# BinFuPKU/CollaborativeFilteringUsingTensorflow

Hardware: AMD Instinct MI355X
Metric: BPR triplets/sec/GPU (d=64) + achieved HBM GB/s; NDCG@10 vs ref (higher is better)
Workload: dtype f32

## Files before the change

collaborativefilteringusingtensorflow_amd/csrc/cf_device.h:

```cpp
#pragma once
#include <hip/hip_runtime.h>
#include <stdint.h>
#include "cf_kernels.h"

namespace cfk {

__host__ __device__ __forceinline__ uint64_t mix64(uint64_t z) {
    z += 0x9E3779B97F4A7C15ull;
    z = (z ^ (z >> 30)) * 0xBF58476D1CE4E5B9ull;
    z = (z ^ (z >> 27)) * 0x94D049BB133111EBull;
    return z ^ (z >> 31);
}

__device__ __forceinline__ uint64_t uniform_below(uint64_t h, uint64_t n) {
    return __umul64hi(h, n);
}

__host__ __device__ __forceinline__ uint64_t perm_rounds(uint64_t x, const PermKey& p) {
#pragma unroll
    for (int r = 0; r < 3; ++r) {
        x = (x ^ p.k[r]) & p.mask;
        x = (x * p.m[r]) & p.mask;
        x ^= x >> p.shift;
    }
    return x;
}

__host__ __device__ __forceinline__ uint64_t permute(uint64_t x, const PermKey& p) {
    do {
        x = perm_rounds(x, p);
    } while (x >= p.n);
    return x;
}

struct PermInv {
    uint64_t mi[3];
};
__host__ __device__ __forceinline__ uint64_t perm_mul_inverse(uint64_t m) {
// ... 87 lines not shown
```

collaborativefilteringusingtensorflow_amd/csrc/cf_engine.cpp:

```cpp
#include <hip/hip_runtime.h>

#include <algorithm>
#include <atomic>
#include <cmath>
#include <cstdio>
#include <cstring>
#include <string>
#include <utility>
#include <vector>

#include "../../include/cf_engine.h"
#include "cf_device.h"
#include "cf_host.h"
#include "cf_kernels.h"
#include <thread>

using namespace cfk;
using namespace cfi;

namespace {
thread_local std::string g_err;
}

std::atomic<int64_t> cfi::g_live_bytes[2];
// ... 27 lines not shown
    int64_t nnz = 0;
    DevBuf<int64_t> indptr;
    DevBuf<int32_t> indices;
    DevBuf<int4> pairs;
    int spec_neg = 0;
    DevBuf<long long> slotP64;
    DevBuf<unsigned long long> GU64;
    DevBuf<int32_t> hotU;
    DevBuf<int> hot_n;
    DevBuf<unsigned long long> GV64;
    int fx_cap = 0;
    DevBuf<unsigned long long> pos_set;
    uint64_t pos_mask = 0;
    int neg_check = 0;
    int64_t nnz_set = 0;
    DevBuf<int64_t> indptr_t;
    DevBuf<int32_t> indices_t;
    std::vector<int64_t> h_indptr;
    int sorted_batches = 2;
    bool sorted_auto_off = false;
    int64_t sorted_reserve_mb = 1024;
    int epoch_sort = 0;
    int user_runs = 0;
    struct EpochOrder {
        DevBuf<int32_t> keys;
        DevBuf<int32_t> vals;
        DevBuf<char> tmp;
        int64_t epoch = -1;
        int B = 0;
        const int32_t* order = nullptr;
        DevBuf<int4> recs;
        const int4* recs_sorted = nullptr;
        bool with_recs = false;
        hipEvent_t ready = nullptr;
        bool async = false;
    } eo[2];
    hipStream_t eo_stream = nullptr;
    hipEvent_t eo_mark = nullptr;

    DevBuf<float> tab[6];
    float *U = nullptr, *V = nullptr, *b = nullptr;
    float *AU = nullptr, *AV = nullptr, *Ab = nullptr;
    DevBuf<float> GU, GV_own, Gb_own;
    float *GV = nullptr, *Gb = nullptr;
    DevBuf<float> GadvU, GadvV;
    float* GadvV_bound = nullptr;
    DevBuf<float> slotU;
    DevBuf<float> slotV;
    DevBuf<float> slotVb;
    int capU = 2, capV = 32;
    bool capU_auto = true;
    int item_recs = 0;
    DevBuf<int4> recV;
    DevBuf<int4> recVc;
    DevBuf<float> stashU, stashB;
    DevBuf<float> GVrep;
// ... 452 lines not shown
            a.fx_bad = e->fx_bad + std::min(e->fx_step++, kFxSlots - 1);
        }
    }
    a.shard_u0 = e->shard_u0;
    a.shard_u1 = e->shard_u1;
    a.plr_kind = c.plr_kind;
    a.alpha = c.alpha;
    a.beta = c.beta;
    a.gamma = c.gamma;
    a.train_bias = (c.model == CF_GBPR || (c.model == CF_PLR && c.plr_kind == CF_PLR_CPLR)) ? 1 : 0;
    a.coefs = e->coefs;
    a.xrows = e->x_rows;
    a.xgrads = e->x_grads;
    return a;
}

constexpr int64_t kSortedAutoBatches = 16;
bool sorted_batches_on(const cf_engine* e, int B) {
    if (e->sorted_batches == 0 || e->nnz > INT32_MAX || B < 1) return false;
    if (e->sorted_batches == 2 && e->sorted_auto_off) return false;
    return e->sorted_batches == 1 || e->sorted_batches == 3 || e->nnz / B >= kSortedAutoBatches;
}

struct EpochNeed {
    bool counting;
    int64_t keys, vals, recs;
    size_t tmp;
    double bytes() const { return 4.0 * (double)(keys + vals) + 16.0 * (double)recs + (double)tmp; }
};
EpochNeed epoch_need(const cf_engine* e, int B) {
    const int64_t nnz = e->nnz;
    const bool wr = e->sorted_batches != 3;
    EpochNeed n{};
    n.counting = e->epoch_sort == 0 && epoch_count_ok(nnz, B);
    if (n.counting) {
        n.recs = wr ? nnz : 0;
        n.vals = wr ? 0 : nnz;
        n.tmp = epoch_count_scratch(nnz, B);
    } else {
        n.keys = 2 * nnz;
        n.recs = wr ? 2 * nnz : 0;
        n.vals = wr ? 0 : 2 * nnz;
        n.tmp = wr ? epoch_records_scratch(nnz, (int32_t)(nnz / B)) : epoch_order_scratch(nnz, (int32_t)(nnz / B));
    }
    return n;
}
// ... 27 lines not shown
        (void)hipGetLastError();
        return true;
    }
    return (double)free_b >= more + (double)e->sorted_reserve_mb * (double)(1 << 20);
}

template <typename T>
int refit(DevBuf<T>& b, size_t need, const char* what) {
    if (b.cap >= need) return CF_OK;
    CF_HIP(hipDeviceSynchronize());
    return b.reset(need, what);
}

int compute_epoch_order(cf_engine* e, int k, int64_t epoch, int B, hipStream_t st) {
    cf_engine::EpochOrder& o = e->eo[k];
    const int64_t nnz = e->nnz;
    const bool wr = e->sorted_batches != 3;
    const EpochNeed n = epoch_need(e, B);
    CF_TRY(refit(o.keys, (size_t)n.keys, "epoch order keys"));
    CF_TRY(refit(o.vals, (size_t)n.vals, "epoch order values"));
    CF_TRY(refit(o.recs, (size_t)n.recs, "epoch order records"));
    CF_TRY(refit(o.tmp, n.tmp, "epoch order scratch"));
    const PermKey pk = make_perm_key((uint64_t)nnz, e->cfg.seed, (uint64_t)epoch);
    {
        ProfScope ps(e, CF_K_EPOCH_ORDER, st);
        if (n.counting) {
            CF_HIP(launch_epoch_count(pk, nnz, B, wr ? e->pairs.p : nullptr, wr ? o.recs.p : nullptr,
                                      wr ? nullptr : o.vals.p, o.tmp, o.tmp.cap, st));
            o.recs_sorted = wr ? o.recs.p : nullptr;
            o.order = wr ? nullptr : o.vals.p;
        } else if (wr) {
            CF_HIP(launch_epoch_records(pk, nnz, B, e->pairs, o.keys, o.recs, o.tmp, o.tmp.cap, &o.recs_sorted, st));
            o.order = nullptr;
        } else {
            CF_HIP(launch_epoch_order(pk, nnz, B, o.keys, o.vals, o.tmp, o.tmp.cap, &o.order, st));
            o.recs_sorted = nullptr;
        }
        o.with_recs = wr;
    }
    o.epoch = epoch;
    o.B = B;
    o.async = st != e->stream;
    if (o.async) CF_HIP(hipEventRecord(o.ready, st));
    return CF_OK;
}

int epoch_order(cf_engine* e, int B, const int32_t** out, const int4** recs_out) {
    if (!e->eo_stream) {
        int lo = 0, hi = 0;
        CF_HIP(hipDeviceGetStreamPriorityRange(&lo, &hi));
        CF_HIP(hipStreamCreateWithPriority(&e->eo_stream, hipStreamNonBlocking, lo));
        CF_HIP(hipEventCreateWithFlags(&e->eo_mark, hipEventDisableTiming));
        for (auto& o : e->eo) CF_HIP(hipEventCreateWithFlags(&o.ready, hipEventDisableTiming));
    }
    const int64_t ep = e->epoch;
    const bool wr = e->sorted_batches != 3;
    auto have = [&](const cf_engine::EpochOrder& o, int64_t epc) { return o.epoch == epc && o.B == B && o.with_recs == wr; };
    int k = have(e->eo[0], ep) ? 0 : have(e->eo[1], ep) ? 1 : -1;
    if (k < 0) {
        k = have(e->eo[0], ep + 1) ? 1 : 0;
        if (e->eo[k].async) CF_HIP(hipStreamWaitEvent(e->stream, e->eo[k].ready, 0));
        CF_HIP(hipEventRecord(e->eo_mark, e->side));
        CF_HIP(hipStreamWaitEvent(e->stream, e->eo_mark, 0));
        CF_TRY(compute_epoch_order(e, k, ep, B, e->stream));
        CF_HIP(hipEventRecord(e->eo_mark, e->stream));
        CF_HIP(hipStreamWaitEvent(e->side, e->eo_mark, 0));
    } else if (e->eo[k].async) {
        CF_HIP(hipStreamWaitEvent(e->stream, e->eo[k].ready, 0));
        CF_HIP(hipStreamWaitEvent(e->side, e->eo[k].ready, 0));
        e->eo[k].async = false;
    }
    *out = e->eo[k].order;
    *recs_out = e->eo[k].with_recs ? e->eo[k].recs_sorted : nullptr;
    cf_engine::EpochOrder& nx = e->eo[k ^ 1];
    if (!have(nx, ep + 1) && e->nnz / B >= 2) {
        CF_HIP(hipEventRecord(e->eo_mark, e->stream));
        CF_HIP(hipStreamWaitEvent(e->eo_stream, e->eo_mark, 0));
        CF_HIP(hipEventRecord(e->eo_mark, e->side));
        CF_HIP(hipStreamWaitEvent(e->eo_stream, e->eo_mark, 0));
        CF_TRY(compute_epoch_order(e, k ^ 1, ep + 1, B, e->eo_stream));
    }
    return CF_OK;
}

int sampler_args(cf_engine* e, int B, StepArgs* a) {
    if (!e->pairs) return fail(CF_ESTATE, "no interactions: call cf_set_interactions first");
    if ((int64_t)B > e->nnz) return fail(CF_EINVAL, "batch size exceeds the number of interactions");
    if (e->full_row_user >= 0)
        return fail(CF_EINVAL, "user " + std::to_string(e->full_row_user) +
                                   " has every item as a positive; the device sampler cannot draw a negative");
    if (e->sampler_B != B) {
        if (e->sampler_B != 0 && e->batch != 0) {
            e->epoch += 1;
            e->batch = 0;
        }
        e->sampler_B = B;
    }
    const int64_t per_epoch = e->nnz / B;
    if (e->batch >= per_epoch) {
        e->epoch += 1;
        e->batch = 0;
    }
    a->sample = 1;
    a->slot_base = (uint64_t)(e->batch * (int64_t)B);
    a->perm = make_perm_key((uint64_t)e->nnz, e->cfg.seed, (uint64_t)e->epoch);
    a->rng_key = mix64_host(e->cfg.seed ^ mix64_host((uint64_t)e->epoch * 0x9E3779B97F4A7C15ull +
                                                     0x2545F4914F6CDD1Dull));
    if (sorted_batches_on(e, B) && e->sorted_batches == 2 && !sorted_auto_fits(e, B)) e->sorted_auto_off = true;
    if (sorted_batches_on(e, B)) {
        const int32_t* ord = nullptr;
        const int4* recs = nullptr;
        const int rc = epoch_order(e, B, &ord, &recs);
        if (rc == CF_ENOMEM && e->sorted_batches == 2) {
            free_epoch_orders(e);
            e->sorted_auto_off = true;
        } else if (rc != CF_OK) {
            return rc;
        } else {
            a->order = ord;
            a->order_recs = recs;
            a->user_runs = e->user_runs && group_count(e->cfg) == 0 ? 1 : 0;
        }
    }
    e->batch += 1;
    return CF_OK;
}

static bool is_device_ptr(const void* p) {
    if (!p) return false;
    hipPointerAttribute_t attr;
    if (hipPointerGetAttributes(&attr, p) != hipSuccess) {
        (void)hipGetLastError();
        return false;
    }
    return attr.type == hipMemoryTypeDevice;
}

static int stage_device_batch(cf_engine* e, const int32_t* pairs, const int32_t* negs,
                       const int32_t* groups, int B, int k, hipStream_t st) {
    const cf_config& c = e->cfg;
    const int W = c.n_neg, G = group_count(c);
    if (!is_device_ptr(negs) || (G > 0 && !is_device_ptr(groups)))
        return fail(CF_EINVAL, "a batch must be all host or all device memory");
// ... 1912 lines not shown
        if (value < 0 || value > 2) return fail(CF_EINVAL, "topk_path must be 0, 1 or 2");
        e->topk_path = (int)value;
        return CF_OK;
    }
    if (n == "item_pieces") {
        if (value < 1 || value > 64) return fail(CF_EINVAL, "item_pieces must be 1 .. 64");
        if (e->lg_stage != 0) return fail(CF_ESTATE, "a split step is in progress");
        e->item_pieces = (int)value;
        return CF_OK;
    }
    if (n == "sorted_batches") {
        if (value < 0 || value > 3) return fail(CF_EINVAL, "sorted_batches must be 0, 1, 2 or 3");
        CF_TRY(discard_pending(e));
        e->sorted_batches = (int)value;
        e->sorted_auto_off = false;
        return CF_OK;
    }
    if (n == "user_runs") {
        if (value < 0 || value > 1) return fail(CF_EINVAL, "user_runs must be 0 or 1");
        CF_TRY(discard_pending(e));
        e->user_runs = (int)value;
        return CF_OK;
    }
    if (n == "epoch_sort") {
        if (value < 0 || value > 1) return fail(CF_EINVAL, "epoch_sort must be 0 or 1");
        CF_TRY(discard_pending(e));
        if (e->eo_stream) CF_HIP(hipStreamSynchronize(e->eo_stream));
        e->epoch_sort = (int)value;
        for (auto& o : e->eo) o.epoch = -1;
        return CF_OK;
    }
    if (n == "sorted_auto_reserve_mb") {
        if (value < 0) return fail(CF_EINVAL, "sorted_auto_reserve_mb must be >= 0");
        CF_TRY(discard_pending(e));
        e->sorted_reserve_mb = value;
        e->sorted_auto_off = false;
        return CF_OK;
    }
    if (n == "spec_neg") {
        if (value < 0 || value > 1) return fail(CF_EINVAL, "spec_neg must be 0 or 1");
        CF_TRY(discard_pending(e));
        e->spec_neg = (int)value;
        return CF_OK;
    }
    if (n == "pair_prefetch") {
        if (value != 0) return fail(CF_EINVAL, "pair_prefetch must be 0 (the prefetch was removed)");
// ... 123 lines not shown
}

int cf_step_path(cf_engine* e, int32_t B, int32_t* flags_out) {
    if (!e || !flags_out) return fail(CF_EINVAL, "null argument");
    if (B < 1) return fail(CF_EINVAL, "B must be >= 1");
    const cf_config& c = e->cfg;
    StepArgs a{};
    a.model = c.model;
    a.d = c.n_factors;
    a.W = c.n_neg;
    a.G = group_count(c);
    a.grad_path = e->grad_path;
    a.apr = (c.model == CF_AMF && e->phase == 1 && c.amf_mode == CF_AMF_APR) ? 1 : 0;
    a.B = B;
    const int kind = grad_plan(a, nullptr).kind;
    int f = 0;
    if (kind == kGradPhased || kind == kGradLds) f |= CF_PATH_PHASED;
    if (psort_active(e, B)) f |= CF_PATH_POS_SORT;
    else if (kind == kGradLds) f |= CF_PATH_LDS;
    if (e->item_recs && (!c.dense_item_apply || e->item_reduce)) f |= CF_PATH_ITEM_RECORDS;
    if (e->det) f |= CF_PATH_DETERMINISTIC;
    if (c.dense_item_apply) f |= CF_PATH_DENSE_ITEMS;
    if (e->pairs && sorted_batches_on(e, B)) f |= CF_PATH_SORTED_BATCHES;
    f |= (e->pipeline & 3) << 8;
    *flags_out = f;
    return CF_OK;
}

int cf_profile_enable(cf_engine* e, int32_t on) {
    if (!e) return fail(CF_EINVAL, "null engine");
    e->prof = on != 0;
    return CF_OK;
}

int cf_profile_read(cf_engine* e, int32_t kid, double* total_ms, int64_t* launches) {
    CF_TRY(check_engine(e));
    if (kid < 0 || kid >= CF_K_COUNT) return fail(CF_EINVAL, "bad kernel id");
    CF_HIP(hipStreamSynchronize(e->stream));
    double t = 0.0;
    for (auto& pr : e->ev[kid]) {
        float ms = 0.f;
        CF_HIP(hipEventSynchronize(pr.second));
        CF_HIP(hipEventElapsedTime(&ms, pr.first, pr.second));
        t += ms;
    }
    if (total_ms) *total_ms = t;
// ... 26 lines not shown
```

collaborativefilteringusingtensorflow_amd/csrc/cf_epoch.hip:

```cpp
#include "cf_kernels.h"
#include "cf_device.h"

namespace cfk {

namespace {

constexpr int kEpochTile = 2048;
constexpr int kEpochItems = kEpochTile / kBlock;
constexpr int kEpochWaveSpan = kEpochTile / kWavesPerBlock;
constexpr int kEpochChunkTiles = 32;

struct EpochCtx {
    uint32_t n, mask, shift, B;
    uint32_t k[3], mi[3];
    uint64_t magic;
    uint32_t nb, n_used;
    int32_t n_bins, nbits;
    int32_t xs_steps;
    int32_t pad;
    int64_t n_tiles;
};

__device__ __forceinline__ uint32_t rounds_inv32(uint32_t q, const EpochCtx& c) {
#pragma unroll
// ... 78 lines not shown
    const int64_t t0 = (int64_t)blockIdx.x * kEpochChunkTiles;
    const int64_t t1 = min(t0 + (int64_t)kEpochChunkTiles, c.n_tiles);
    for (int b = threadIdx.x; b < c.n_bins; b += kBlock) {
        int32_t run = csum[(int64_t)blockIdx.x * c.n_bins + b];
        for (int64_t g = t0; g < t1; ++g) {
            const int32_t t = cnt[g * c.n_bins + b];
            cnt[g * c.n_bins + b] = run;
            run += t;
        }
    }
}

__device__ __forceinline__ int32_t block_excl_scan(int32_t v, int32_t* wtot) {
    const int w = threadIdx.x >> 6, lane = threadIdx.x & 63;
    const int32_t inc = wave_incl_scan(v);
    if (lane == kWave - 1) wtot[w] = inc;
    __syncthreads();
    int32_t before = 0;
#pragma unroll
    for (int i = 0; i < kWavesPerBlock; ++i) before += i < w ? wtot[i] : 0;
    return before + inc - v;
}

template <bool RECS>
__global__ void __launch_bounds__(kBlock) epoch_scatter_kernel(EpochCtx c, const uint16_t* __restrict__ bins,
                                                               const int32_t* __restrict__ off,
                                                               const int4* __restrict__ pairs,
                                                               int4* __restrict__ out_recs,
                                                               int32_t* __restrict__ out_idx) {
    extern __shared__ int32_t lds[];
    const int nbn = c.n_bins;
    int32_t* stage = lds;
    int32_t* gstage = stage + kEpochTile;
    int32_t* wtot = gstage + kEpochTile;
    int32_t* wcnt = wtot + kWavesPerBlock;
    int32_t* delta = wcnt + kWavesPerBlock * nbn;
    const int tid = threadIdx.x, w = tid >> 6, lane = tid & 63;
    const uint32_t tile0 = (uint32_t)blockIdx.x * kEpochTile;
    const uint32_t qend = min(tile0 + (uint32_t)kEpochTile, c.n);
    const int tile_len = (int)(qend - tile0);
    for (int b = tid; b < kWavesPerBlock * nbn; b += kBlock) wcnt[b] = 0;
    __syncthreads();
    const uint32_t w0 = tile0 + (uint32_t)(w * kEpochWaveSpan);
    constexpr int KC = kEpochWaveSpan / kWave;
    int key[KC];
#pragma unroll
    for (int k = 0; k < KC; ++k) {
        const uint32_t q = w0 + (uint32_t)(k * kWave + lane);
        key[k] = q < qend ? (int)bins[q] : nbn;
    }
#pragma unroll
    for (int k = 0; k < KC; ++k)
// ... 38 lines not shown
        for (int bit = 0; bit < c.nbits; ++bit) {
            const bool s = (key[k] >> bit) & 1;
            const uint64_t m = __ballot(s);
            peers &= s ? m : ~m;
        }
        const int rank = __popcll(peers & below);
        if (key[k] < nbn) {
            const int32_t lp = pos[key[k]] + rank;
            if (rank == 0) pos[key[k]] = lp + __popcll(peers);
            gstage[lp] = lp + delta[key[k]];
            stage[lp] = (int32_t)(w0 + (uint32_t)(k * kWave + lane));
        }
    }
    __syncthreads();
    if (RECS) {
        int4 r[kEpochItems];
        int32_t g[kEpochItems];
#pragma unroll
        for (int i = 0; i < kEpochItems; ++i) {
            const int L = tid + i * kBlock;
            const int Lc = L < tile_len ? L : 0;
            g[i] = gstage[Lc];
            r[i] = pairs[stage[Lc]];
        }
        __builtin_amdgcn_sched_barrier(0);
#pragma unroll
        for (int i = 0; i < kEpochItems; ++i) out_recs[g[i]] = r[i];
    } else {
#pragma unroll
        for (int i = 0; i < kEpochItems; ++i) {
            const int L = tid + i * kBlock;
            if (L < tile_len) out_idx[gstage[L]] = stage[L];
        }
    }
}

EpochCtx epoch_ctx(const PermKey& p, int64_t nnz, int B) {
    EpochCtx c{};
    c.n = (uint32_t)p.n;
    c.mask = (uint32_t)p.mask;
    c.shift = p.shift;
    c.B = (uint32_t)B;
    for (int r = 0; r < 3; ++r) {
        c.k[r] = (uint32_t)p.k[r];
        c.mi[r] = (uint32_t)perm_mul_inverse(p.m[r]);
    }
// ... 12 lines not shown
    c.n_tiles = (nnz + kEpochTile - 1) / kEpochTile;
    return c;
}

int64_t n_chunks_of(int64_t n_tiles) { return (n_tiles + kEpochChunkTiles - 1) / kEpochChunkTiles; }

size_t align16(size_t x) { return (x + 15) & ~(size_t)15; }

}

bool epoch_count_ok(int64_t nnz, int B) {
    return nnz > 0 && nnz <= INT32_MAX && B > 0 && nnz / B + 1 <= kEpochMaxBins;
}

size_t epoch_count_scratch(int64_t nnz, int B) {
    if (!epoch_count_ok(nnz, B)) return 0;
    const int64_t n_bins = nnz / B + 1;
    const int64_t n_tiles = (nnz + kEpochTile - 1) / kEpochTile;
    return align16((size_t)nnz * sizeof(uint16_t)) +
           (size_t)((n_tiles + n_chunks_of(n_tiles)) * n_bins) * sizeof(int32_t);
}

hipError_t launch_epoch_count(const PermKey& p, int64_t nnz, int B, const int4* pairs, int4* out_recs,
                              int32_t* out_idx, void* tmp, size_t tmp_bytes, hipStream_t s) {
    if (!epoch_count_ok(nnz, B) || (uint64_t)nnz != p.n || p.mask > 0xFFFFFFFFull) return hipErrorInvalidValue;
    if ((pairs == nullptr) != (out_recs == nullptr) || (out_recs == nullptr) == (out_idx == nullptr))
        return hipErrorInvalidValue;
    if (tmp_bytes < epoch_count_scratch(nnz, B)) return hipErrorInvalidValue;
    const EpochCtx c = epoch_ctx(p, nnz, B);
    const int64_t n_chunks = n_chunks_of(c.n_tiles);
    uint16_t* bins = static_cast<uint16_t*>(tmp);
    int32_t* cnt = reinterpret_cast<int32_t*>(static_cast<char*>(tmp) + align16((size_t)nnz * sizeof(uint16_t)));
    int32_t* csum = cnt + c.n_tiles * c.n_bins;
    const dim3 grid((unsigned)c.n_tiles);
    const size_t lds1 = (size_t)c.n_bins * sizeof(int32_t) + kEpochTile * sizeof(uint16_t);
    hipLaunchKernelGGL(epoch_bins_kernel, grid, dim3(kBlock), lds1, s, c, bins, cnt);
    hipLaunchKernelGGL(epoch_chunk_sum_kernel, dim3((unsigned)n_chunks), dim3(kBlock), 0, s, c, cnt, csum);
    hipLaunchKernelGGL(epoch_chunk_scan_kernel, dim3((unsigned)((c.n_bins + kWavesPerBlock - 1) / kWavesPerBlock)),
                       dim3(kBlock), 0, s, c, csum, n_chunks);
    hipLaunchKernelGGL(epoch_tile_offsets_kernel, dim3((unsigned)n_chunks), dim3(kBlock), 0, s, c, cnt, csum);
    size_t lds3 = (size_t)(kWavesPerBlock + 1) * c.n_bins * sizeof(int32_t) +
                  (size_t)(2 * kEpochTile + kWavesPerBlock) * sizeof(int32_t);
    if (out_recs)
        hipLaunchKernelGGL(epoch_scatter_kernel<true>, grid, dim3(kBlock), lds3, s, c, bins, cnt, pairs, out_recs,
                           nullptr);
    else
        hipLaunchKernelGGL(epoch_scatter_kernel<false>, grid, dim3(kBlock), lds3, s, c, bins, cnt, nullptr, nullptr,
                           out_idx);
    return hipGetLastError();
}

}
```

collaborativefilteringusingtensorflow_amd/csrc/cf_kernels.h:

```cpp
#pragma once
#include <hip/hip_runtime.h>
#include <stdint.h>

namespace cfk {

constexpr int kWave = 64;
constexpr int kBlock = 256;
constexpr int kWavesPerBlock = kBlock / kWave;
constexpr int kGL = 16;
constexpr int kGroupsPerBlock = kBlock / kGL;
#ifndef CF_PAIRS_PER_GROUP
#define CF_PAIRS_PER_GROUP 2
#endif
constexpr int kPairsPerGroup = CF_PAIRS_PER_GROUP;
constexpr int kPairsPerBlock = kGroupsPerBlock * kPairsPerGroup;
constexpr int kMaxNeg = 64;
constexpr int kMaxGroup = 16;
constexpr int kMaxFactors = 256;

enum Model { BPR = 0, GBPR = 1, CML = 2, AMF = 3, PLR = 4 };

struct PermKey {
    uint64_t n;
    uint64_t mask;
// ... 20 lines not shown
    int apr_embed_done;
    int use_rank_weight;
    float n_items_f;
    int64_t n_items;
    float lr, clip_norm;
    int clip;
    int sample;
    int count_users;
    int count_items;
    int items_grad_only;
    uint64_t slot_base;
    uint64_t rng_key;
    PermKey perm;
    const int4* __restrict__ pairs;
    const int64_t* __restrict__ indptr;
    const int32_t* __restrict__ indices;
    const int64_t* __restrict__ indptr_t;
    const int32_t* __restrict__ indices_t;
    const unsigned long long* __restrict__ pos_set;
    uint64_t pos_mask;
    const int32_t* __restrict__ order;
    const int4* __restrict__ order_recs;
    int user_runs;
    int det_fx;
    long long* __restrict__ slotP64;
    unsigned long long* __restrict__ GU64;
    const int32_t* __restrict__ hotU;
    unsigned long long* __restrict__ GV64;
    int* __restrict__ fx_bad;
    int2* __restrict__ spec_ph;
    int* __restrict__ spec_n;
    float* __restrict__ U; float* __restrict__ AU; float* __restrict__ GU;
    float* __restrict__ V; float* __restrict__ AV; float* __restrict__ GV;
    float* __restrict__ b; float* __restrict__ Ab; float* __restrict__ Gb;
    int32_t* __restrict__ occU;
    int32_t* __restrict__ occV;
    int32_t* __restrict__ cntU;
    int32_t* __restrict__ cntV;
    int32_t* __restrict__ rankU;
    int32_t* __restrict__ rankV;
    float* __restrict__ slotU;
    float* __restrict__ slotV;
    int capU, capV;
    float* __restrict__ GVrep;
    int repV;
    const int32_t* __restrict__ offU;
// ... 248 lines not shown
    const int32_t* occV; const int32_t* rankV;
    const int32_t* cntU;
    int32_t* hotU;
    int* hot_n;
    const int32_t* cntV; const int32_t* cntP;
    int2* offPN;
    int32_t* srec;
    int B, W, capU;
    int64_t n_items;
    const int2* spec_ph;
    const int* spec_n;
    float* slotN;
    int32_t* cntVw;
    int d;
};
hipError_t launch_psort(const PsortArgs& a, void* tmp, size_t tmp_bytes, hipStream_t s);
size_t epoch_order_scratch(int64_t nnz, int32_t n_batches);
hipError_t launch_epoch_order(const PermKey& p, int64_t nnz, int B, int32_t* keys, int32_t* vals, void* tmp,
                              size_t tmp_bytes, const int32_t** order_out, hipStream_t s);
size_t epoch_records_scratch(int64_t nnz, int32_t n_batches);
hipError_t launch_epoch_records(const PermKey& p, int64_t nnz, int B, const int4* pairs, int32_t* keys, int4* recs,
                                void* tmp, size_t tmp_bytes, const int4** recs_out, hipStream_t s);
constexpr int kEpochMaxBins = 1024;
bool epoch_count_ok(int64_t nnz, int B);
size_t epoch_count_scratch(int64_t nnz, int B);
hipError_t launch_epoch_count(const PermKey& p, int64_t nnz, int B, const int4* pairs, int4* out_recs,
                              int32_t* out_idx, void* tmp, size_t tmp_bytes, hipStream_t s);
hipError_t launch_uncount_spec(const int2* ph, int* n, int32_t* cnt, hipStream_t s);
hipError_t launch_build_pos_set(const int4* pairs, int64_t nnz, unsigned long long* set,
                                uint64_t mask, hipStream_t s);
hipError_t launch_build_pairs(const int64_t* indptr, const int32_t* indices, int64_t n_users,
                              int4* pairs, hipStream_t s);
hipError_t launch_score(const ScoreArgs& a, hipStream_t s);
hipError_t launch_topk(const TopkArgs& a, int n_users, hipStream_t s);
hipError_t launch_fused_topk(const FusedTopkArgs& a, hipStream_t s);
hipError_t launch_xchg_pack(const XchgArgs& a, hipStream_t s);
hipError_t launch_xchg_serve(const int32_t* ids, int64_t n, int64_t u0, int32_t* cntU, int32_t* own,
                             const float* U, float* rows, int d, hipStream_t s);
hipError_t launch_xchg_accumulate(const int32_t* ids, int64_t n, int64_t u0, const float* grads,
                                  float* GU, int d, hipStream_t s);

PermKey make_perm_key(uint64_t n, uint64_t seed, uint64_t epoch);
uint64_t mix64_host(uint64_t z);

}
```

collaborativefilteringusingtensorflow_amd/csrc/cf_kernels.hip:

```cpp
#include "cf_kernels_impl.h"

namespace cfk {

__global__ void init_normal_kernel(float* __restrict__ X, int64_t n, float mean, float stddev,
                                   int truncated, uint64_t seed) {
    const int64_t t0 = (int64_t)blockIdx.x * blockDim.x + threadIdx.x;
    const int64_t nt = (int64_t)gridDim.x * blockDim.x;
    for (int64_t k = t0; k < n; k += nt) {
        uint64_t ctr = 0;
        float z;
        do {
            const uint64_t h = mix64(seed ^ mix64((uint64_t)k * 0x9E3779B97F4A7C15ull + ctr++));
            const float u1 = ((uint32_t)(h >> 40) + 0.5f) * (1.f / 16777216.f);
            const float u2 = ((uint32_t)(h & 0xFFFFFF)) * (1.f / 16777216.f);
            z = sqrtf(-2.f * logf(u1)) * cospif(2.f * u2);
        } while (truncated && fabsf(z) > 2.f);
        X[k] = mean + stddev * z;
    }
}

__global__ void fill_kernel(float* __restrict__ X, int64_t n, float v) {
    const int64_t t0 = (int64_t)blockIdx.x * blockDim.x + threadIdx.x;
    const int64_t nt = (int64_t)gridDim.x * blockDim.x;
    for (int64_t k = t0; k < n; k += nt) X[k] = v;
// ... 438 lines not shown
        const int32_t g = a.g[(int64_t)p * a.gs + k];
        int32_t v;
        if (a.sharded) {
            const bool gok = g >= 0 && g < a.total_users;
            ok = ok && gok;
            v = !gok ? 0 : (g >= a.shard_u0 && g < a.shard_u1) ? (int32_t)(g - a.shard_u0) : -1 - g;
        } else {
            const bool gok = g >= 0 && g < a.n_users;
            ok = ok && gok;
            v = gok ? g : 0;
        }
        a.occU[a.B + (int64_t)p * a.G + k] = v;
    }
    if (!ok) atomicMin(a.bad, p);
}

hipError_t launch_pack_batch(const PackArgs& a, hipStream_t s) {
    if (a.B <= 0) return hipSuccess;
    hipLaunchKernelGGL(pack_batch_kernel, dim3((a.B + kBlock - 1) / kBlock), dim3(kBlock), 0, s, a);
    return hipGetLastError();
}

uint64_t mix64_host(uint64_t z) { return mix64(z); }

PermKey make_perm_key(uint64_t n, uint64_t seed, uint64_t epoch) {
    PermKey p{};
    p.n = n;
    uint32_t bits = 1;
    while (bits < 63 && (1ull << bits) < n) ++bits;
    p.mask = (1ull << bits) - 1ull;
    p.shift = bits / 2 > 0 ? bits / 2 : 1;
    uint64_t h = mix64(seed ^ mix64(epoch + 0x5851F42D4C957F2Dull));
    for (int r = 0; r < 3; ++r) {
        h = mix64(h + (uint64_t)r);
        p.k[r] = h & p.mask;
        p.m[r] = (mix64(h ^ 0xA0761D6478BD642Full) | 1ull);
    }
    return p;
}

hipError_t launch_det_hot(const HotArgs& h, hipStream_t s) {
    const int64_t ntiles = h.n / kDetTile;
    if (ntiles <= 0) return hipSuccess;
    const dim3 grid((unsigned)(ntiles < 16384 ? ntiles : 16384)), block(kBlock);
    return with_epl(h.d, [&](auto e) {
        hipLaunchKernelGGL(det_hot_kernel<decltype(e)::value>, grid, block, 0, s, h);
// ... 5 lines not shown
```

collaborativefilteringusingtensorflow_amd/csrc/cf_kernels_impl.h:

```cpp
#pragma once
#include <algorithm>
#include <type_traits>

#include "cf_kernels.h"
#include "cf_device.h"

#ifndef CF_PREP_GL
#define CF_PREP_GL 8
#endif
#ifndef CF_PREP_CHUNKS
#define CF_PREP_CHUNKS 8
#endif
#ifndef CF_PREP_GL_W1
#define CF_PREP_GL_W1 4
#endif
#ifndef CF_PREP_CHUNKS_W1
#define CF_PREP_CHUNKS_W1 (64 / CF_PREP_GL_W1)
#endif
#ifndef CF_SORT_MIN_WAVES
#define CF_SORT_MIN_WAVES 1
#endif
#ifndef CF_SORT_TILES
#define CF_SORT_TILES 1
#endif
#ifndef CF_LDS_WAVES
#define CF_LDS_WAVES 1
#endif
#ifndef CF_LDS_WAVES_GBPR
#define CF_LDS_WAVES_GBPR 1
#endif
#ifndef CF_APPLY_NF
#define CF_APPLY_NF 4
#endif
#ifndef CF_APPLY_NF_PS
#define CF_APPLY_NF_PS 8
#endif
#ifndef CF_APPLY_MIN_WAVES
#define CF_APPLY_MIN_WAVES 1
#endif
#ifndef CF_APPLY_DETECT_WAVES
// ... 262 lines not shown
        unsafeAtomicAdd(a.Gb + r, g);
    }
}

__device__ __forceinline__ void bias_finish_pre(const StepArgs& a, int64_t r, int count, float g,
                                                int64_t slot, float b0, float ab0) {
    if (count == 1 && !a.items_grad_only) {
        const float acc = fmaf(g, g, ab0);
        a.Ab[r] = acc;
        a.b[r] = b0 - adagrad_delta(a.lr, g, acc);
    } else {
        bias_finish(a, r, count, g, slot);
    }
}

__device__ __forceinline__ float neg_log_sigmoid(float x) {
    return -logf(rcp_1p(expf(-x)));
}

__device__ __forceinline__ float softplus(float x) {
    return x > 0.f ? x + log1pf(expf(-x)) : log1pf(expf(x));
}

__device__ __forceinline__ int32_t draw_item(uint64_t key, uint64_t ctr, int64_t n_items) {
    return (int32_t)uniform_below(mix64(key + ctr), (uint64_t)n_items);
}

constexpr int kPrepGL = CF_PREP_GL;
constexpr int kPrepPairsPerBlock = kBlock / kPrepGL;
constexpr int kPrepChunks = CF_PREP_CHUNKS;
__host__ __device__ constexpr int prep_chunks(int pgl) { return pgl == kPrepGL ? kPrepChunks : CF_PREP_CHUNKS_W1; }

template <int PGL = kPrepGL>
__device__ __forceinline__ uint32_t gor8(uint32_t v) {
    if constexpr (PGL == 4 || PGL == 8) {
        v |= dpp_u<0xB1>(v);
        v |= dpp_u<0x4E>(v);
        if constexpr (PGL == 8) v |= dpp_u<0x141>(v);
        return v;
    }
#pragma unroll
    for (int o = PGL / 2; o >= 1; o >>= 1) v |= (uint32_t)__shfl_xor((int)v, o, 64);
    return v;
}
template <int PGL>
__device__ __forceinline__ int32_t gbcast(int32_t v, int k) {
    if constexpr (PGL == 4) {
        switch (k) {
            case 0: return (int32_t)dpp_u<0x00>((uint32_t)v);
            case 1: return (int32_t)dpp_u<0x55>((uint32_t)v);
// ... 42 lines not shown
                hit |= (c < ncand && el[q] == cand[c]) ? (1u << c) : 0u;
    }
    return hit;
}

template <int MODEL, int PGL = kPrepGL>
__device__ __forceinline__ void prep_body(const StepArgs& a, int block) {
    const int gl = threadIdx.x & (PGL - 1);
    const int p = block * (kBlock / PGL) + (threadIdx.x / PGL);
    if (p >= a.B) return;
    const int W = a.W;
    const int G = (MODEL == GBPR) ? a.G : 0;
    const int B = a.B;
    int u, i;
    uint64_t key = 0;
    int64_t rb = 0, re = 0;
    if (a.sample) {
        const uint64_t slot = a.slot_base + (uint64_t)p;
        const int4 pr = a.order_recs != nullptr ? a.order_recs[slot]
                      : a.order != nullptr    ? a.pairs[a.order[slot]]
                                              : a.pairs[permute(slot, a.perm)];
        u = pr.x;
        i = pr.y;
        key = mix64(a.rng_key ^ (slot * 0xD1B54A32D192ED03ull));
        rb = (int64_t)(uint32_t)pr.z;
        re = rb + pr.w;
    } else {
        u = a.occU[p];
        i = a.occV[p];
    }
    const bool runs = a.user_runs != 0 && a.sample && a.count_users;
    int run_rank = 0, run_len = 0, run_lead = 0, run_base = 0;
    bool run_atomic = false;
    if (runs) {
        constexpr int GPW = kWave / PGL;
        const int lane = threadIdx.x & 63, lead = lane & ~(PGL - 1), g = lane / PGL;
        const int uprev = __shfl_up(u, PGL, kWave), unext = __shfl_down(u, PGL, kWave);
        const bool head = g == 0 || uprev != u;
        const bool tail = g == GPW - 1 || p + 1 >= B || unext != u;
        const uint64_t H = __ballot(gl == 0 && head), T = __ballot(gl == 0 && tail);
        const uint64_t hm = H & ((2ull << lead) - 1ull);
        const uint64_t tm = T & ~((1ull << lead) - 1ull);
        run_lead = 63 - __clzll((long long)hm);
        const int last = __ffsll((unsigned long long)tm) - 1;
        run_rank = (lead - run_lead) / PGL;
        run_len = (last - run_lead) / PGL + 1;
        run_atomic = run_lead == 0 || last == (GPW - 1) * PGL;
// ... 77 lines not shown
            if (a.sample) {
                const int64_t cb = a.indptr_t[i], ce = a.indptr_t[i + 1];
                const uint64_t h = mix64(key + ((uint64_t)(kMaxNeg + k) << 32));
                g = a.indices_t[cb + (int64_t)uniform_below(h, (uint64_t)(ce - cb))];
                g = (g >= a.shard_u0 && g < a.shard_u1) ? g - a.shard_u0 : -1 - g;
                a.occU[B + p * G + k] = g;
            } else {
                g = a.occU[B + p * G + k];
            }
            if (a.count_users && g >= 0) a.rankU[B + p * G + k] = atomicAdd(&a.cntU[g], 1);
        }
    }
    if (runs) rk_u = __shfl(run_base, run_lead, kWave) + run_rank;
    if (gl == 0) {
        if (a.sample) {
            a.occU[p] = u;
            a.occV[p] = i;
        }
        if (a.count_users) a.rankU[p] = rk_u;
        if (a.count_items) a.rankV[p] = rk_i;
    }
}

template <int MODEL>
__device__ __forceinline__ void prep_any(const StepArgs& a, int block) {
    if (a.W == 1)
        prep_body<MODEL, CF_PREP_GL_W1>(a, block);
    else
        prep_body<MODEL>(a, block);
}

__host__ __device__ __forceinline__ int prep_pairs_per_block(const StepArgs& a) {
    return a.W == 1 ? kBlock / CF_PREP_GL_W1 : kPrepPairsPerBlock;
}

template <int MODEL>
__global__ __launch_bounds__(kBlock) void prep_kernel(StepArgs a) {
    prep_any<MODEL>(a, blockIdx.x);
}

template <int EPL, int WT>
struct NegRows {
    static constexpr int N = WT > 0 ? WT : 1;
    int j[N];
    int c[N];
    int64_t sl[N];
    float v[N][EPL];
    __device__ __forceinline__ void prefetch(const StepArgs& a, int p, int gl) {
        if constexpr (WT > 0) {
            int rk[N];
#pragma unroll
            for (int w = 0; w < WT; ++w) {
                j[w] = a.occV[a.B + p * WT + w];
                rk[w] = a.count_items ? a.rankV[a.B + p * WT + w] : 0;
            }
// ... 2006 lines not shown
```

collaborativefilteringusingtensorflow_amd/engine.py:

```python
import ctypes

import numpy as np

from . import _native as N
from ._native import _ptr


def _i32(a):
    return np.ascontiguousarray(a, dtype=np.int32)


def _is_dev(x):
    return hasattr(x, "data_ptr") and bool(getattr(x, "is_cuda", False))


def _dev(t, dtype, ctype):
    import torch
    t = t.to(dtype).contiguous()
    torch.cuda.current_stream(t.device).synchronize()
    return t, ctypes.cast(t.data_ptr(), ctypes.POINTER(ctype))


class _DevArg(object):

# ... 485 lines not shown
        if _is_dev(users):
            import torch
            u, up = _dev(users.reshape(-1), torch.int32, ctypes.c_int32)
            n = u.shape[0]
            rows = torch.empty((n, cut.shape[0], 7), dtype=torch.float64, device=u.device) if per_user else None
            lists = torch.empty((n, max(k, 0)), dtype=torch.int32, device=u.device) if return_lists else None
            uptr = ctypes.c_void_p(u.data_ptr())
            rp = ctypes.c_void_p(rows.data_ptr()) if per_user else None
            lp = ctypes.c_void_p(lists.data_ptr()) if return_lists else None
        else:
            u = _i32(users).reshape(-1)
            n = u.shape[0]
            rows = np.empty((n, cut.shape[0], 7), dtype=np.float64) if per_user else None
            lists = np.empty((n, max(k, 0)), dtype=np.int32) if return_lists else None
            uptr = ctypes.c_void_p(u.ctypes.data)
            rp = ctypes.c_void_p(rows.ctypes.data) if per_user else None
            lp = ctypes.c_void_p(lists.ctypes.data) if return_lists else None
        N.check(self._L.cf_evaluate(self._h, uptr, n, cp, int(cut.shape[0]), 1 if exclude_train else 0, mp,
                                    sp, rp, lp), "cf_evaluate")
        out = (sums,) + ((rows,) if per_user else ()) + ((lists,) if return_lists else ())
        return out if len(out) > 1 else sums

    PATH_FLAGS = {"phased": 1, "pos_sort": 2, "item_records": 4, "deterministic": 8, "dense_items": 16,
                  "lds": 32, "sorted_batches": 64}

    def step_path(self, batch_size):
        f = ctypes.c_int32(0)
        N.check(self._L.cf_step_path(self._h, int(batch_size), ctypes.byref(f)), "cf_step_path")
        v = int(f.value)
        out = {k: bool(v & m) for k, m in self.PATH_FLAGS.items()}
        out["pipeline"] = (v >> 8) & 3
        return v, out

    def set_option(self, name, value):
        N.check(self._L.cf_set_option(self._h, name.encode(), int(value)), "cf_set_option(%s)" % name)

    def profile(self, on=True):
        N.check(self._L.cf_profile_enable(self._h, 1 if on else 0), "cf_profile_enable")

    def profile_read(self, kernel):
        ms, n = ctypes.c_double(0.0), ctypes.c_int64(0)
        N.check(self._L.cf_profile_read(self._h, N.KERNELS[kernel], ctypes.byref(ms),
                                        ctypes.byref(n)), "cf_profile_read")
        return float(ms.value), int(n.value)

    def profile_reset(self):
        N.check(self._L.cf_profile_reset(self._h), "cf_profile_reset")
# ... 44 lines not shown
```

include/cf_engine.h:

```cpp
#ifndef CF_ENGINE_H
#define CF_ENGINE_H

#include <stdint.h>

#ifdef __cplusplus
extern "C" {
#endif

#define CF_ABI_VERSION 1

typedef struct cf_engine cf_engine;

enum cf_model {
    CF_BPR = 0,
    CF_GBPR = 1,
    CF_CML = 2,
    CF_AMF = 3,
    CF_PLR = 4
};

enum cf_plr_kind {
    CF_PLR_PRIGP = 0,
    CF_PLR_CPLR = 1
};
// ... 124 lines not shown
                        const void* grad_bias);
int cf_bind_table(cf_engine* eng, int32_t table, void* device_ptr, int64_t n_elems);
int cf_set_shard(cf_engine* eng, int32_t world, int32_t rank, const int64_t* user_bounds );
int cf_set_group_source(cf_engine* eng, const int64_t* indptr_t, const int32_t* indices_t, int64_t nnz);
int cf_bind_exchange(cf_engine* eng, void* send_ids, void* rows, void* grads, int64_t send_cap,
                     void* recv_ids, void* serve_rows, void* serve_grads, int64_t recv_cap);
int cf_xchg_begin(cf_engine* eng, int32_t B, const int32_t* host_pairs, const int32_t* host_negs,
                  const int32_t* host_groups, int32_t* send_counts_out);
int cf_xchg_draw(cf_engine* eng, int32_t B, void* send_counts_dev, int32_t* half_out);
int cf_xchg_adopt(cf_engine* eng, int32_t B);
int cf_xchg_serve(cf_engine* eng, int64_t n_recv);
int cf_xchg_grad(cf_engine* eng);
int cf_xchg_grad_part(cf_engine* eng, int32_t part);
int cf_xchg_finish_items(cf_engine* eng);
int cf_xchg_finish(cf_engine* eng, int64_t n_recv);

enum cf_path_flag {
    CF_PATH_PHASED = 1,
    CF_PATH_POS_SORT = 2,
    CF_PATH_ITEM_RECORDS = 4,
    CF_PATH_DETERMINISTIC = 8,
    CF_PATH_DENSE_ITEMS = 16,
    CF_PATH_LDS = 32,
    CF_PATH_SORTED_BATCHES = 64
};
int cf_step_path(cf_engine* eng, int32_t B, int32_t* flags_out);

int cf_take_loss(cf_engine* eng, double* loss_sum_out);

int cf_step_plr(cf_engine* eng, const int32_t* host_tuples, int32_t width, const float* host_coefs,
                int32_t B, double* loss_out);

int cf_score_topk(cf_engine* eng, const int32_t* host_users, int32_t n,
                  int32_t k, const uint8_t* mask_or_NULL, int32_t* host_idx_out,
                  float* host_val_out);
int cf_score_topk_ex(cf_engine* eng, const int32_t* host_users, int32_t n,
                     int32_t k, int32_t exclude_train, const uint8_t* item_mask,
                     int32_t* host_idx_out, float* host_val_out);

enum { CF_EVAL_PRE = 0, CF_EVAL_RECALL = 1, CF_EVAL_NDCG = 2, CF_EVAL_MAP = 3, CF_EVAL_MRR = 4,
       CF_EVAL_HR = 5, CF_EVAL_ARHR = 6, CF_EVAL_N = 7 };
int cf_set_truth(cf_engine* eng, const int64_t* indptr , const int32_t* indices, int64_t nnz);
int cf_eval_lists(cf_engine* eng, const int32_t* users, int32_t n, const int32_t* idx , int32_t k,
                  const int32_t* cutoffs, int32_t n_cut,
                  double* sums_out , double* per_user_out_or_NULL );
int cf_evaluate(cf_engine* eng, const int32_t* users, int32_t n, const int32_t* cutoffs, int32_t n_cut,
                int32_t exclude_train, const uint8_t* item_mask,
// ... 110 lines not shown
```

Baseline: 1.559 billion.

## Draw BPR negatives during epoch-order scatter and store them in records

```diff
diff --git a/collaborativefilteringusingtensorflow_amd/csrc/cf_device.h b/collaborativefilteringusingtensorflow_amd/csrc/cf_device.h
--- a/collaborativefilteringusingtensorflow_amd/csrc/cf_device.h
+++ b/collaborativefilteringusingtensorflow_amd/csrc/cf_device.h
@@ -14,6 +14,16 @@
 
 __device__ __forceinline__ uint64_t uniform_below(uint64_t h, uint64_t n) {
     return __umul64hi(h, n);
+}
+
+__host__ __device__ __forceinline__ uint64_t draw_rng_key(uint64_t seed, uint64_t epoch) {
+    return mix64(seed ^ mix64(epoch * 0x9E3779B97F4A7C15ull + 0x2545F4914F6CDD1Dull));
+}
+__host__ __device__ __forceinline__ uint64_t draw_pair_key(uint64_t rng_key, uint64_t slot) {
+    return mix64(rng_key ^ (slot * 0xD1B54A32D192ED03ull));
+}
+__device__ __forceinline__ int32_t draw_item(uint64_t key, uint64_t ctr, int64_t n_items) {
+    return (int32_t)uniform_below(mix64(key + ctr), (uint64_t)n_items);
 }
 
 __host__ __device__ __forceinline__ uint64_t perm_rounds(uint64_t x, const PermKey& p) {
diff --git a/collaborativefilteringusingtensorflow_amd/csrc/cf_engine.cpp b/collaborativefilteringusingtensorflow_amd/csrc/cf_engine.cpp
--- a/collaborativefilteringusingtensorflow_amd/csrc/cf_engine.cpp
+++ b/collaborativefilteringusingtensorflow_amd/csrc/cf_engine.cpp
@@ -73,6 +73,7 @@
     int64_t sorted_reserve_mb = 1024;
     int epoch_sort = 0;
     int user_runs = 0;
+    int neg_records = 2;
     struct EpochOrder {
         DevBuf<int32_t> keys;
         DevBuf<int32_t> vals;
@@ -83,6 +84,7 @@
         DevBuf<int4> recs;
         const int4* recs_sorted = nullptr;
         bool with_recs = false;
+        bool with_negs = false;
         hipEvent_t ready = nullptr;
         bool async = false;
     } eo[2];
@@ -581,6 +583,14 @@
     return e->sorted_batches == 1 || e->sorted_batches == 3 || e->nnz / B >= kSortedAutoBatches;
 }
 
+bool neg_records_on(const cf_engine* e, int B) {
+    const cf_config& c = e->cfg;
+    if (e->neg_records == 0 || !e->pairs || !sorted_batches_on(e, B) || e->sorted_batches == 3) return false;
+    if (e->epoch_sort != 0 || !epoch_count_ok(e->nnz, B)) return false;
+    if (c.model == CF_PLR || c.n_neg != 1 || group_count(c) != 0) return false;
+    return !e->neg_check && !e->spec_neg && !e->user_runs;
+}
+
 struct EpochNeed {
     bool counting;
     int64_t keys, vals, recs;
@@ -654,11 +664,13 @@
     CF_TRY(refit(o.recs, (size_t)n.recs, "epoch order records"));
     CF_TRY(refit(o.tmp, n.tmp, "epoch order scratch"));
     const PermKey pk = make_perm_key((uint64_t)nnz, e->cfg.seed, (uint64_t)epoch);
+    const bool wn = neg_records_on(e, B);
+    const EpochNeg neg{e->indices.p, e->cfg.n_items, draw_rng_key_host(e->cfg.seed, (uint64_t)epoch)};
     {
         ProfScope ps(e, CF_K_EPOCH_ORDER, st);
         if (n.counting) {
             CF_HIP(launch_epoch_count(pk, nnz, B, wr ? e->pairs.p : nullptr, wr ? o.recs.p : nullptr,
-                                      wr ? nullptr : o.vals.p, o.tmp, o.tmp.cap, st));
+                                      wr ? nullptr : o.vals.p, o.tmp, o.tmp.cap, st, wn ? &neg : nullptr));
             o.recs_sorted = wr ? o.recs.p : nullptr;
             o.order = wr ? nullptr : o.vals.p;
         } else if (wr) {
@@ -669,6 +681,7 @@
             o.recs_sorted = nullptr;
         }
         o.with_recs = wr;
+        o.with_negs = wn;
     }
     o.epoch = epoch;
     o.B = B;
@@ -677,7 +690,7 @@
     return CF_OK;
 }
 
-int epoch_order(cf_engine* e, int B, const int32_t** out, const int4** recs_out) {
+int epoch_order(cf_engine* e, int B, const int32_t** out, const int4** recs_out, int* negs_out) {
     if (!e->eo_stream) {
         int lo = 0, hi = 0;
         CF_HIP(hipDeviceGetStreamPriorityRange(&lo, &hi));
@@ -687,7 +700,10 @@
     }
     const int64_t ep = e->epoch;
     const bool wr = e->sorted_batches != 3;
-    auto have = [&](const cf_engine::EpochOrder& o, int64_t epc) { return o.epoch == epc && o.B == B && o.with_recs == wr; };
+    const bool wn = neg_records_on(e, B);
+    auto have = [&](const cf_engine::EpochOrder& o, int64_t epc) {
+        return o.epoch == epc && o.B == B && o.with_recs == wr && o.with_negs == wn;
+    };
     int k = have(e->eo[0], ep) ? 0 : have(e->eo[1], ep) ? 1 : -1;
     if (k < 0) {
         k = have(e->eo[0], ep + 1) ? 1 : 0;
@@ -704,6 +720,7 @@
     }
     *out = e->eo[k].order;
     *recs_out = e->eo[k].with_recs ? e->eo[k].recs_sorted : nullptr;
+    *negs_out = e->eo[k].with_recs && e->eo[k].with_negs ? 1 : 0;
     cf_engine::EpochOrder& nx = e->eo[k ^ 1];
     if (!have(nx, ep + 1) && e->nnz / B >= 2) {
         CF_HIP(hipEventRecord(e->eo_mark, e->stream));
@@ -736,21 +753,23 @@
     a->sample = 1;
     a->slot_base = (uint64_t)(e->batch * (int64_t)B);
     a->perm = make_perm_key((uint64_t)e->nnz, e->cfg.seed, (uint64_t)e->epoch);
-    a->rng_key = mix64_host(e->cfg.seed ^ mix64_host((uint64_t)e->epoch * 0x9E3779B97F4A7C15ull +
-                                                     0x2545F4914F6CDD1Dull));
+    a->rng_key = draw_rng_key_host(e->cfg.seed, (uint64_t)e->epoch);
     if (sorted_batches_on(e, B) && e->sorted_batches == 2 && !sorted_auto_fits(e, B)) e->sorted_auto_off = true;
     if (sorted_batches_on(e, B)) {
         const int32_t* ord = nullptr;
         const int4* recs = nullptr;
-        const int rc = epoch_order(e, B, &ord, &recs);
+        int negs = 0;
+        const int rc = epoch_order(e, B, &ord, &recs, &negs);
         if (rc == CF_ENOMEM && e->sorted_batches == 2) {
             free_epoch_orders(e);
+            (void)hipGetLastError();
             e->sorted_auto_off = true;
         } else if (rc != CF_OK) {
             return rc;
         } else {
             a->order = ord;
             a->order_recs = recs;
+            a->neg_recs = negs;
             a->user_runs = e->user_runs && group_count(e->cfg) == 0 ? 1 : 0;
         }
     }
@@ -2709,6 +2728,12 @@
         e->user_runs = (int)value;
         return CF_OK;
     }
+    if (n == "neg_records") {
+        if (value < 0 || value > 2) return fail(CF_EINVAL, "neg_records must be 0, 1 or 2");
+        CF_TRY(discard_pending(e));
+        e->neg_records = (int)value;
+        return CF_OK;
+    }
     if (n == "epoch_sort") {
         if (value < 0 || value > 1) return fail(CF_EINVAL, "epoch_sort must be 0 or 1");
         CF_TRY(discard_pending(e));
@@ -2878,6 +2903,7 @@
     if (e->det) f |= CF_PATH_DETERMINISTIC;
     if (c.dense_item_apply) f |= CF_PATH_DENSE_ITEMS;
     if (e->pairs && sorted_batches_on(e, B)) f |= CF_PATH_SORTED_BATCHES;
+    if (neg_records_on(e, B)) f |= CF_PATH_NEG_RECORDS;
     f |= (e->pipeline & 3) << 8;
     *flags_out = f;
     return CF_OK;
diff --git a/collaborativefilteringusingtensorflow_amd/csrc/cf_epoch.hip b/collaborativefilteringusingtensorflow_amd/csrc/cf_epoch.hip
--- a/collaborativefilteringusingtensorflow_amd/csrc/cf_epoch.hip
+++ b/collaborativefilteringusingtensorflow_amd/csrc/cf_epoch.hip
@@ -124,12 +124,12 @@
     return before + inc - v;
 }
 
-template <bool RECS>
+template <bool RECS, bool NEG = false>
 __global__ void __launch_bounds__(kBlock) epoch_scatter_kernel(EpochCtx c, const uint16_t* __restrict__ bins,
                                                                const int32_t* __restrict__ off,
                                                                const int4* __restrict__ pairs,
                                                                int4* __restrict__ out_recs,
-                                                               int32_t* __restrict__ out_idx) {
+                                                               int32_t* __restrict__ out_idx, EpochNeg neg) {
     extern __shared__ int32_t lds[];
     const int nbn = c.n_bins;
     int32_t* stage = lds;
@@ -214,6 +214,48 @@
             const int Lc = L < tile_len ? L : 0;
             g[i] = gstage[Lc];
             r[i] = pairs[stage[Lc]];
+        }
+        if constexpr (NEG) {
+            const int32_t* __restrict__ ind = neg.indices;
+            int32_t j[kEpochItems];
+            uint32_t found = 0;
+#pragma unroll
+            for (int i = 0; i < kEpochItems; ++i)
+                j[i] = draw_item(draw_pair_key(neg.rng_key, (uint64_t)(uint32_t)g[i]), 0, neg.n_items);
+            bool more = true;
+            while (more) {
+                more = false;
+#pragma unroll
+                for (int i = 0; i < kEpochItems; ++i) {
+                    if (r[i].w > 0) {
+                        const int32_t half = r[i].w >> 1;
+                        const int32_t v = ind[(uint32_t)r[i].z + (uint32_t)half];
+                        if (v < j[i]) {
+                            r[i].z += half + 1;
+                            r[i].w -= half + 1;
+                        } else {
+                            r[i].w = v == j[i] ? 0 : half;
+                        }
+                        found |= v == j[i] ? 1u << i : 0u;
+                        more |= r[i].w > 0;
+                    }
+                }
+            }
+#pragma unroll
+            for (int i = 0; i < kEpochItems; ++i) {
+                if ((found >> i) & 1u) {
+                    const int L = tid + i * kBlock;
+                    const int4 q = pairs[stage[L < tile_len ? L : 0]];
+                    const int64_t rb = (int64_t)(uint32_t)q.z, re = rb + q.w;
+                    const uint64_t key = draw_pair_key(neg.rng_key, (uint64_t)(uint32_t)g[i]);
+                    uint64_t k = 1;
+                    do {
+                        j[i] = draw_item(key, k++, neg.n_items);
+                    } while (sorted_contains(ind, rb, re, j[i]));
+                }
+                r[i].z = j[i];
+                r[i].w = 0;
+            }
         }
         __builtin_amdgcn_sched_barrier(0);
 #pragma unroll
@@ -272,9 +314,11 @@
 }
 
 hipError_t launch_epoch_count(const PermKey& p, int64_t nnz, int B, const int4* pairs, int4* out_recs,
-                              int32_t* out_idx, void* tmp, size_t tmp_bytes, hipStream_t s) {
+                              int32_t* out_idx, void* tmp, size_t tmp_bytes, hipStream_t s, const EpochNeg* neg) {
     if (!epoch_count_ok(nnz, B) || (uint64_t)nnz != p.n || p.mask > 0xFFFFFFFFull) return hipErrorInvalidValue;
     if ((pairs == nullptr) != (out_recs == nullptr) || (out_recs == nullptr) == (out_idx == nullptr))
+        return hipErrorInvalidValue;
+    if (neg != nullptr && (out_recs == nullptr || neg->indices == nullptr || neg->n_items < 1))
         return hipErrorInvalidValue;
     if (tmp_bytes < epoch_count_scratch(nnz, B)) return hipErrorInvalidValue;
     const EpochCtx c = epoch_ctx(p, nnz, B);
@@ -291,12 +335,15 @@
     hipLaunchKernelGGL(epoch_tile_offsets_kernel, dim3((unsigned)n_chunks), dim3(kBlock), 0, s, c, cnt, csum);
     size_t lds3 = (size_t)(kWavesPerBlock + 1) * c.n_bins * sizeof(int32_t) +
                   (size_t)(2 * kEpochTile + kWavesPerBlock) * sizeof(int32_t);
-    if (out_recs)
-        hipLaunchKernelGGL(epoch_scatter_kernel<true>, grid, dim3(kBlock), lds3, s, c, bins, cnt, pairs, out_recs,
-                           nullptr);
+    if (neg)
+        hipLaunchKernelGGL((epoch_scatter_kernel<true, true>), grid, dim3(kBlock), lds3, s, c, bins, cnt, pairs,
+                           out_recs, nullptr, *neg);
+    else if (out_recs)
+        hipLaunchKernelGGL((epoch_scatter_kernel<true>), grid, dim3(kBlock), lds3, s, c, bins, cnt, pairs, out_recs,
+                           nullptr, EpochNeg{});
     else
-        hipLaunchKernelGGL(epoch_scatter_kernel<false>, grid, dim3(kBlock), lds3, s, c, bins, cnt, nullptr, nullptr,
-                           out_idx);
+        hipLaunchKernelGGL((epoch_scatter_kernel<false>), grid, dim3(kBlock), lds3, s, c, bins, cnt, nullptr, nullptr,
+                           out_idx, EpochNeg{});
     return hipGetLastError();
 }
 
diff --git a/collaborativefilteringusingtensorflow_amd/csrc/cf_kernels.h b/collaborativefilteringusingtensorflow_amd/csrc/cf_kernels.h
--- a/collaborativefilteringusingtensorflow_amd/csrc/cf_kernels.h
+++ b/collaborativefilteringusingtensorflow_amd/csrc/cf_kernels.h
@@ -66,6 +66,7 @@
     const int32_t* __restrict__ order;
     const int4* __restrict__ order_recs;
     int user_runs;
+    int neg_recs;
     int det_fx;
     long long* __restrict__ slotP64;
     unsigned long long* __restrict__ GU64;
@@ -360,10 +361,16 @@
 hipError_t launch_epoch_records(const PermKey& p, int64_t nnz, int B, const int4* pairs, int32_t* keys, int4* recs,
                                 void* tmp, size_t tmp_bytes, const int4** recs_out, hipStream_t s);
 constexpr int kEpochMaxBins = 1024;
+struct EpochNeg {
+    const int32_t* indices;
+    int64_t n_items;
+    uint64_t rng_key;
+};
 bool epoch_count_ok(int64_t nnz, int B);
 size_t epoch_count_scratch(int64_t nnz, int B);
 hipError_t launch_epoch_count(const PermKey& p, int64_t nnz, int B, const int4* pairs, int4* out_recs,
-                              int32_t* out_idx, void* tmp, size_t tmp_bytes, hipStream_t s);
+                              int32_t* out_idx, void* tmp, size_t tmp_bytes, hipStream_t s,
+                              const EpochNeg* neg = nullptr);
 hipError_t launch_uncount_spec(const int2* ph, int* n, int32_t* cnt, hipStream_t s);
 hipError_t launch_build_pos_set(const int4* pairs, int64_t nnz, unsigned long long* set,
                                 uint64_t mask, hipStream_t s);
@@ -380,5 +387,6 @@
 
 PermKey make_perm_key(uint64_t n, uint64_t seed, uint64_t epoch);
 uint64_t mix64_host(uint64_t z);
+uint64_t draw_rng_key_host(uint64_t seed, uint64_t epoch);
 
 }
diff --git a/collaborativefilteringusingtensorflow_amd/csrc/cf_kernels.hip b/collaborativefilteringusingtensorflow_amd/csrc/cf_kernels.hip
--- a/collaborativefilteringusingtensorflow_amd/csrc/cf_kernels.hip
+++ b/collaborativefilteringusingtensorflow_amd/csrc/cf_kernels.hip
@@ -484,6 +484,7 @@
 }
 
 uint64_t mix64_host(uint64_t z) { return mix64(z); }
+uint64_t draw_rng_key_host(uint64_t seed, uint64_t epoch) { return draw_rng_key(seed, epoch); }
 
 PermKey make_perm_key(uint64_t n, uint64_t seed, uint64_t epoch) {
     PermKey p{};
diff --git a/collaborativefilteringusingtensorflow_amd/csrc/cf_kernels_impl.h b/collaborativefilteringusingtensorflow_amd/csrc/cf_kernels_impl.h
--- a/collaborativefilteringusingtensorflow_amd/csrc/cf_kernels_impl.h
+++ b/collaborativefilteringusingtensorflow_amd/csrc/cf_kernels_impl.h
@@ -16,6 +16,9 @@
 #endif
 #ifndef CF_PREP_CHUNKS_W1
 #define CF_PREP_CHUNKS_W1 (64 / CF_PREP_GL_W1)
+#endif
+#ifndef CF_PREP_GL_REC
+#define CF_PREP_GL_REC 1
 #endif
 #ifndef CF_SORT_MIN_WAVES
 #define CF_SORT_MIN_WAVES 1
@@ -324,10 +327,6 @@
     return x > 0.f ? x + log1pf(expf(-x)) : log1pf(expf(x));
 }
 
-__device__ __forceinline__ int32_t draw_item(uint64_t key, uint64_t ctr, int64_t n_items) {
-    return (int32_t)uniform_below(mix64(key + ctr), (uint64_t)n_items);
-}
-
 constexpr int kPrepGL = CF_PREP_GL;
 constexpr int kPrepPairsPerBlock = kBlock / kPrepGL;
 constexpr int kPrepChunks = CF_PREP_CHUNKS;
@@ -416,7 +415,7 @@
                                               : a.pairs[permute(slot, a.perm)];
         u = pr.x;
         i = pr.y;
-        key = mix64(a.rng_key ^ (slot * 0xD1B54A32D192ED03ull));
+        key = draw_pair_key(a.rng_key, slot);
         rb = (int64_t)(uint32_t)pr.z;
         re = rb + pr.w;
     } else {
@@ -540,15 +539,42 @@
     }
 }
 
+template <int LPP>
+__device__ __forceinline__ void prep_recs_body(const StepArgs& a, int block) {
+    static_assert(LPP == 1 || LPP == 2 || LPP == 4, "lanes per pair of the record draw");
+    const int gl = threadIdx.x & (LPP - 1);
+    const int p = block * (kBlock / LPP) + (threadIdx.x / LPP);
+    if (p >= a.B) return;
+    const int4 pr = a.order_recs[a.slot_base + (uint64_t)p];
+    const int32_t id[3] = {pr.x, pr.y, pr.z};
+    int32_t* const cnt[3] = {a.cntU, a.cntP != nullptr ? a.cntP : a.cntV, a.cntV};
+    const bool count[3] = {a.count_users != 0, a.count_items != 0, a.count_items != 0};
+    int32_t* const occ[3] = {a.occU + p, a.occV + p, a.occV + a.B + p};
+    int32_t* const rank[3] = {a.rankU + p, a.rankV + p, a.rankV + a.B + p};
+    int32_t rk[3] = {0, 0, 0};
+#pragma unroll
+    for (int k = 0; k < 3; ++k)
+        if ((k & (LPP - 1)) == gl && count[k]) rk[k] = atomicAdd(&cnt[k][id[k]], 1);
+#pragma unroll
+    for (int k = 0; k < 3; ++k)
+        if ((k & (LPP - 1)) == gl) *occ[k] = id[k];
+#pragma unroll
+    for (int k = 0; k < 3; ++k)
+        if ((k & (LPP - 1)) == gl && count[k]) *rank[k] = rk[k];
+}
+
 template <int MODEL>
 __device__ __forceinline__ void prep_any(const StepArgs& a, int block) {
-    if (a.W == 1)
+    if (a.neg_recs)
+        prep_recs_body<CF_PREP_GL_REC>(a, block);
+    else if (a.W == 1)
         prep_body<MODEL, CF_PREP_GL_W1>(a, block);
     else
         prep_body<MODEL>(a, block);
 }
 
 __host__ __device__ __forceinline__ int prep_pairs_per_block(const StepArgs& a) {
+    if (a.neg_recs) return kBlock / CF_PREP_GL_REC;
     return a.W == 1 ? kBlock / CF_PREP_GL_W1 : kPrepPairsPerBlock;
 }
 
diff --git a/collaborativefilteringusingtensorflow_amd/engine.py b/collaborativefilteringusingtensorflow_amd/engine.py
--- a/collaborativefilteringusingtensorflow_amd/engine.py
+++ b/collaborativefilteringusingtensorflow_amd/engine.py
@@ -531,7 +531,7 @@
         return out if len(out) > 1 else sums
 
     PATH_FLAGS = {"phased": 1, "pos_sort": 2, "item_records": 4, "deterministic": 8, "dense_items": 16,
-                  "lds": 32, "sorted_batches": 64}
+                  "lds": 32, "sorted_batches": 64, "neg_records": 128}
 
     def step_path(self, batch_size):
         f = ctypes.c_int32(0)
diff --git a/include/cf_engine.h b/include/cf_engine.h
--- a/include/cf_engine.h
+++ b/include/cf_engine.h
@@ -170,7 +170,8 @@
     CF_PATH_DETERMINISTIC = 8,
     CF_PATH_DENSE_ITEMS = 16,
     CF_PATH_LDS = 32,
-    CF_PATH_SORTED_BATCHES = 64
+    CF_PATH_SORTED_BATCHES = 64,
+    CF_PATH_NEG_RECORDS = 128
 };
 int cf_step_path(cf_engine* eng, int32_t B, int32_t* flags_out);
 
```

New measurement: 1.636 billion (median of 6 runs). +4.9%, better.
